# Biblbrox/ViT-Spectre-Experiments

Hardware: AMD Instinct MI355X
Metric: images/sec training, Spectre-ViT-S CIFAR-100 bs512 (higher is better)
Workload: dtype bf16

## Files before the change

### vit-spectre-experiments_amd/csrc/spv_rowops.hip

```cpp
#define SPV_USES_SEED
#include "spv_common.h"

namespace {

constexpr float LN_EPS = 1e-5f;
constexpr int RT = 256;
constexpr int RW = RT / 64;
constexpr int BWD_MAX_WG = 1024;

enum PoolMode { POOL_IDENT = 0, POOL_EXACT = 1, POOL_TABLE = 2, POOL_REPEAT = 3 };

template <int VEC> __device__ __forceinline__ void ldv(const void* base, size_t off, int bf, float (&v)[VEC]);
template <> __device__ __forceinline__ void ldv<4>(const void* base, size_t off, int bf, float (&v)[4]) {
    if (bf) io<bf16_t>::ld4(static_cast<const bf16_t*>(base) + off, v);
    else io<float>::ld4(static_cast<const float*>(base) + off, v);
}
template <> __device__ __forceinline__ void ldv<1>(const void* base, size_t off, int bf, float (&v)[1]) {
    v[0] = bf ? bf2f(static_cast<const bf16_t*>(base)[off]) : static_cast<const float*>(base)[off];
}
template <int VEC> __device__ __forceinline__ void stv(void* base, size_t off, int bf, const float (&v)[VEC]);
template <> __device__ __forceinline__ void stv<4>(void* base, size_t off, int bf, const float (&v)[4]) {
    if (bf) io<bf16_t>::st4(static_cast<bf16_t*>(base) + off, v);
    else io<float>::st4(static_cast<float*>(base) + off, v);
}
// ... 680 lines not shown
#pragma unroll
        for (int j = 0; j < KD; ++j) {
            const unsigned w[4] = {raw[j].x, raw[j].y, raw[j].z, raw[j].w};
            const float d0[4] = {__uint_as_float(da[j].x << 16), __uint_as_float(da[j].x & 0xffff0000u), __uint_as_float(da[j].y << 16),
                                 __uint_as_float(da[j].y & 0xffff0000u)};
            const float d1[4] = {__uint_as_float(dd[j].x << 16), __uint_as_float(dd[j].x & 0xffff0000u), __uint_as_float(dd[j].y << 16),
                                 __uint_as_float(dd[j].y & 0xffff0000u)};
#pragma unroll
            for (int u = 0; u < 4; ++u) {
                const float x0 = __uint_as_float(w[u] << 16), x1 = __uint_as_float(w[u] & 0xffff0000u);
                const float a = bf2f(f2bf((x0 + x1) * r)), d = bf2f(f2bf((x0 - x1) * r));
                xh0[j][u] = (a - mu) * rs;
                xh1[j][u] = (d - mu) * rs;
                acc[0][j][u] += d0[u] * xh0[j][u];
                acc[1][j][u] += d0[u];
                acc[0][KD + j][u] += d1[u] * xh1[j][u];
                acc[1][KD + j][u] += d1[u];
                t0[j][u] = d0[u] * g0[j][u];
                t1[j][u] = d1[u] * g1[j][u];
                s1 += t0[j][u] + t1[j][u];
                s2 += t0[j][u] * xh0[j][u] + t1[j][u] * xh1[j][u];
            }
        }
        const float m1 = wave_sum(s1) * (1.0f / (float)D), m2 = wave_sum(s2) * (1.0f / (float)D);
        bf16_t* orow = dx + (size_t)row * D;
#pragma unroll
        for (int j = 0; j < KD; ++j) {
            const int c = 64 * j + lane;
            const unsigned wr[4] = {res[j].x, res[j].y, res[j].z, res[j].w};
            float o[8];
#pragma unroll
            for (int u = 0; u < 4; ++u) {
                const float ga = bf2f(f2bf(rs * (t0[j][u] - m1 - xh0[j][u] * m2)));
                const float gd = bf2f(f2bf(rs * (t1[j][u] - m1 - xh1[j][u] * m2)));
                o[2 * u] = (ga + gd) * r + __uint_as_float(wr[u] << 16);
                o[2 * u + 1] = (ga - gd) * r + __uint_as_float(wr[u] & 0xffff0000u);
            }
            uint4 t;
            t.x = pack_bf16x2(o[0], o[1]); t.y = pack_bf16x2(o[2], o[3]); t.z = pack_bf16x2(o[4], o[5]); t.w = pack_bf16x2(o[6], o[7]);
            *reinterpret_cast<uint4*>(orow + 8 * c) = t;
        }
    }
    write_partials<4, MAXI, 2>(acc, lds, partials + (size_t)blockIdx.x * 2 * D, D, lane, wave);
}

__global__ __launch_bounds__(FOLD_COLS * FOLD_ROWS) void fold_partials_kernel(const float* __restrict__ partials, float* __restrict__ o0,
                                                                             float* __restrict__ o1, float* __restrict__ o2,
                                                                             int parts, int np, int n, float* __restrict__ o3 = nullptr,
                                                                             float* __restrict__ o4 = nullptr) {
    const FoldJob j{partials, {o0, o1, o2, o3, o4}, parts, np, n};
    fold_partials_block(j, blockIdx.x, threadIdx.x);
}

constexpr int lc_ws(int c, int CO, int CI) { return (c * CI) / CO; }
constexpr int lc_we(int c, int CO, int CI) { return ((c + 1) * CI + CO - 1) / CO; }

template <int CNT> __device__ __forceinline__ void ld_span(const void* base, size_t off, int bf, float (&v)[CNT]) {
#pragma unroll
    for (int q = 0; q < CNT / 4; ++q) {
        float t[4];
        ldv<4>(base, off + 4 * q, bf, t);
#pragma unroll
        for (int u = 0; u < 4; ++u) v[4 * q + u] = t[u];
    }
}
template <int CNT> __device__ __forceinline__ void st_span(void* base, size_t off, int bf, const float (&v)[CNT]) {
#pragma unroll
    for (int q = 0; q < CNT / 4; ++q) {
        float t[4];
#pragma unroll
        for (int u = 0; u < 4; ++u) t[u] = v[4 * q + u];
        stv<4>(base, off + 4 * q, bf, t);
    }
}

template <int CNT, int BF> struct RawSpan;
template <int CNT> struct RawSpan<CNT, 1> { unsigned w[CNT / 2]; };
template <int CNT> struct RawSpan<CNT, 0> { float w[CNT]; };
template <int CNT, int BF> __device__ __forceinline__ void ld_raw(const void* base, size_t off, RawSpan<CNT, BF>& r) {
    if constexpr (BF) {
        const unsigned* p = reinterpret_cast<const unsigned*>(static_cast<const bf16_t*>(base) + off);
#pragma unroll
        for (int i = 0; i < CNT / 2; ++i) r.w[i] = p[i];
    } else {
        const float* p = static_cast<const float*>(base) + off;
#pragma unroll
        for (int i = 0; i < CNT; ++i) r.w[i] = p[i];
    }
}
template <int CNT, int BF> __device__ __forceinline__ void unpack(const RawSpan<CNT, BF>& r, float (&v)[CNT]) {
    if constexpr (BF) {
#pragma unroll
        for (int i = 0; i < CNT / 2; ++i) {
            v[2 * i] = __uint_as_float(r.w[i] << 16);
            v[2 * i + 1] = __uint_as_float(r.w[i] & 0xffff0000u);
        }
    } else {
#pragma unroll
        for (int i = 0; i < CNT; ++i) v[i] = r.w[i];
    }
}

struct TailLn2 {
    const void* res;
    const float* gamma2;
    const float* beta2;
    void* out2;
    float* mean2;
    float* rstd2;
    const void* dout2;
    const void* f3;
    void* ds;
};
__device__ __forceinline__ float round_store(float v, int bf) { return bf ? bf2f(f2bf(v)) : v; }

template <int CO, int CI, bool FASTG, bool LN2>
__global__ __launch_bounds__(RT, 4) void tail_fwd_lc_kernel(const void* __restrict__ h, const void* __restrict__ x,
                                                             const float* __restrict__ gamma, const float* __restrict__ beta,
                                                             void* __restrict__ out, float* __restrict__ mean_o,
                                                             float* __restrict__ rstd_o, int rows, int bf_rt, int out_bf_rt, float p_drop,
                                                             uint64_t seed, TailLn2 ln) {
    constexpr int bf = FASTG ? 1 : 0, out_bf = bf;
    (void)bf_rt; (void)out_bf_rt;
    constexpr int n = 64 * CO, k_in = 64 * CI;
    constexpr float inv_n = 1.0f / (float)n;
    const int lane = threadIdx.x & 63;
    const int wave_g = blockIdx.x * RW + (threadIdx.x >> 6);
    const int nwaves = gridDim.x * RW;
    const float inv_keep = p_drop > 0.0f ? 1.0f / (1.0f - p_drop) : 1.0f;
    const uint64_t seed_l = live_seed(seed);
    float g[CO], b[CO];
    ld_span<CO>(gamma, (size_t)lane * CO, 0, g);
    ld_span<CO>(beta, (size_t)lane * CO, 0, b);
    for (int row = wave_g; row < rows; row += nwaves) {
        RawSpan<CO, bf> r_h, r_res;
        RawSpan<CI, bf> r_x;
        ld_raw<CO, bf>(h, (size_t)row * n + lane * CO, r_h);
        ld_raw<CI, bf>(x, (size_t)row * k_in + lane * CI, r_x);
        if (LN2) ld_raw<CO, bf>(ln.res, (size_t)row * n + lane * CO, r_res);
        float hv[CO], xin[CI];
        unpack<CO, bf>(r_h, hv);
        unpack<CI, bf>(r_x, xin);
        float s = 0.0f;
#pragma unroll
        for (int c = 0; c < CO; ++c) s += hv[c];
        const float mean = wave_sum(s) * inv_n;
        float q = 0.0f;
#pragma unroll
        for (int c = 0; c < CO; ++c) { const float d = hv[c] - mean; q += d * d; }
        const float rstd = rsqrtf(wave_sum(q) * inv_n + LN_EPS);
        const unsigned rkey = p_drop > 0.0f ? dropout_row_key(seed_l, (uint64_t)row) : 0u;
        const unsigned lane_gold = (unsigned)(lane * (CO / 2)) * 0x9e3779b1u;
        float o[CO];
#pragma unroll
        for (int c = 0; c < CO; c += 2) {
            float pv[2];
#pragma unroll
            for (int u = 0; u < 2; ++u) {
                float acc = 0.0f;
#pragma unroll
                for (int j = 0; j < CI; ++j)
                    if (j >= lc_ws(c + u, CO, CI) && j < lc_we(c + u, CO, CI)) acc += xin[j];
                pv[u] = acc * (1.0f / (float)(lc_we(c + u, CO, CI) - lc_ws(c + u, CO, CI)));
            }
            const f32x2 hv2 = {hv[c], hv[c + 1]}, g2 = {g[c], g[c + 1]}, b2 = {b[c], b[c + 1]};
            const f32x2 ln = (hv2 - mean) * (g2 * rstd) + b2;
            f32x2 act, unused;
            if (FASTG) gelu_fast2(ln, act, unused);
            else act = f32x2{gelu_erf(ln.x), gelu_erf(ln.y)};
            o[c] = act.x + pv[0];
            o[c + 1] = act.y + pv[1];
            if (p_drop > 0.0f) {
                o[c] *= dropout_scale_at(rkey + lane_gold, c, p_drop, inv_keep);
                o[c + 1] *= dropout_scale_at(rkey + lane_gold, c + 1, p_drop, inv_keep);
            }
        }
        st_span<CO>(out, (size_t)row * n + lane * CO, out_bf, o);
        if (lane == 0) { mean_o[row] = mean; rstd_o[row] = rstd; }
        if (LN2) {
            float rv[CO], g2[CO], b2[CO];
            unpack<CO, bf>(r_res, rv);
            float sm = 0.0f;
#pragma unroll
            for (int c = 0; c < CO; ++c) { rv[c] += round_store(o[c], out_bf); sm += rv[c]; }
            const float mean2 = wave_sum(sm) * inv_n;
            float q2 = 0.0f;
#pragma unroll
            for (int c = 0; c < CO; ++c) { const float d = rv[c] - mean2; q2 += d * d; }
            const float rstd2 = rsqrtf(wave_sum(q2) * inv_n + LN_EPS);
            ld_span<CO>(ln.gamma2, (size_t)lane * CO, 0, g2);
            ld_span<CO>(ln.beta2, (size_t)lane * CO, 0, b2);
#pragma unroll
            for (int c = 0; c < CO; ++c) rv[c] = (rv[c] - mean2) * rstd2 * g2[c] + b2[c];
            st_span<CO>(ln.out2, (size_t)row * n + lane * CO, bf, rv);
            if (lane == 0) { ln.mean2[row] = mean2; ln.rstd2[row] = rstd2; }
        }
    }
}

struct TailUp {
    const void* src;
    float p_drop;
    uint64_t seed;
};

template <int CO, int CI, bool FASTG, bool LN2>
__global__ __launch_bounds__(RT, 4) void tail_bwd_lc_kernel(const void* __restrict__ dout, const void* __restrict__ h,
                                                             const float* __restrict__ mean_i, const float* __restrict__ rstd_i,
                                                             const float* __restrict__ gamma, const float* __restrict__ beta,
                                                             void* __restrict__ dh, void* __restrict__ dxp, float* __restrict__ partials,
                                                             int rows, int bf_rt, int dout_bf_rt, float p_drop, uint64_t seed,
                                                             const void* __restrict__ dx_add, TailLn2 ln, TailUp up) {
    extern __shared__ __attribute__((aligned(16))) float lds[];
    constexpr int bf = FASTG ? 1 : 0;
    (void)bf_rt; (void)dout_bf_rt;
    constexpr int n = 64 * CO, k_in = 64 * CI, Q = CO / 4;
    constexpr float inv_n = 1.0f / (float)n;
    constexpr int NP = LN2 ? 5 : 3;
    static_assert(CO % 4 == 0, "lane span must be whole float4s");
    const int lane = threadIdx.x & 63, wave = threadIdx.x >> 6;
    const int wave_g = blockIdx.x * RW + wave;
    const int nwaves = gridDim.x * RW;
    const float inv_keep = p_drop > 0.0f ? 1.0f / (1.0f - p_drop) : 1.0f;
    float4* accw = reinterpret_cast<float4*>(lds) + (size_t)wave * NP * Q * 64 + lane;
#pragma unroll
    for (int i = 0; i < NP * Q; ++i) accw[i * 64] = make_float4(0.0f, 0.0f, 0.0f, 0.0f);
    const uint64_t seed_l = live_seed(seed), up_seed_l = live_seed(up.seed);
    for (int row = wave_g; row < rows; row += nwaves) {
        RawSpan<CO, bf> r_h, r_d, r_s, r_t;
        RawSpan<CI, bf> r_u, r_a;
        ld_raw<CO, bf>(LN2 ? ln.dout2 : dout, (size_t)row * n + lane * CO, r_d);
        ld_raw<CO, bf>(h, (size_t)row * n + lane * CO, r_h);
        if (LN2) {
            ld_raw<CO, bf>(ln.f3, (size_t)row * n + lane * CO, r_s);
            ld_raw<CO, bf>(ln.res, (size_t)row * n + lane * CO, r_t);
        }
        constexpr bool WIDE_IN = CI > 16;
        if constexpr (!WIDE_IN) {
            if (!LN2 && up.src != nullptr) ld_raw<CI, bf>(up.src, (size_t)row * k_in + lane * CI, r_u);
            if (dxp != nullptr && dx_add != nullptr) ld_raw<CI, bf>(dx_add, (size_t)row * k_in + lane * CI, r_a);
        }
        const float mean = mean_i[row], rstd = rstd_i[row];
        const unsigned rkey = p_drop > 0.0f ? dropout_row_key(seed_l, (uint64_t)row) : 0u;
        const unsigned lane_gold = (unsigned)(lane * (CO / 2)) * 0x9e3779b1u;
        float hv[CO], dv[CO], dxh[CO];
        unpack<CO, bf>(r_d, dv);
        if (LN2) {
            float sv[CO], tv[CO];
            unpack<CO, bf>(r_s, sv);
            unpack<CO, bf>(r_t, tv);
            const float mean2 = ln.mean2[row], rstd2 = ln.rstd2[row];
            float t1 = 0.0f, t2 = 0.0f;
#pragma unroll
            for (int q = 0; q < Q; ++q) {
                float g2[4];
                ld_span<4>(ln.gamma2, (size_t)lane * CO + 4 * q, 0, g2);
                float4 v3 = accw[(3 * Q + q) * 64], v4 = accw[(4 * Q + q) * 64];
                float a3[4];
#pragma unroll
                for (int e = 0; e < 4; ++e) {
                    const int c = 4 * q + e;
                    const float xh = (sv[c] + tv[c] - mean2) * rstd2;
                    a3[e] = dv[c] * xh;
                    sv[c] = xh;
                    tv[c] = dv[c] * g2[e];
                    t1 += tv[c];
                    t2 += tv[c] * xh;
                }
                v3.x += a3[0]; v3.y += a3[1]; v3.z += a3[2]; v3.w += a3[3];
                v4.x += dv[4 * q]; v4.y += dv[4 * q + 1]; v4.z += dv[4 * q + 2]; v4.w += dv[4 * q + 3];
                accw[(3 * Q + q) * 64] = v3;
                accw[(4 * Q + q) * 64] = v4;
            }
            const float n1 = wave_sum(t1) * inv_n, n2 = wave_sum(t2) * inv_n;
#pragma unroll
            for (int c = 0; c < CO; ++c) dv[c] = round_store(rstd2 * (tv[c] - n1 - sv[c] * n2), bf);
            st_span<CO>(ln.ds, (size_t)row * n + lane * CO, bf, dv);
        } else {
            if (up.src != nullptr) {
                float u[CI];
                unpack<CI, bf>(r_u, u);
                if (up.p_drop > 0.0f) {
                    const unsigned ukey = dropout_row_key(up_seed_l, (uint64_t)row);
                    const float uinv = 1.0f / (1.0f - up.p_drop);
#pragma unroll
                    for (int c = 0; c < CI; ++c) u[c] *= dropout_scale_at(ukey + (unsigned)(lane * (CI / 2)) * 0x9e3779b1u, c, up.p_drop, uinv);
                }
#pragma unroll
                for (int j = 0; j < CO; ++j) {
                    float a = 0.0f;
#pragma unroll
                    for (int c = 0; c < CI; ++c)
                        if (j >= lc_ws(c, CI, CO) && j < lc_we(c, CI, CO)) a += u[c] * (1.0f / (float)(lc_we(c, CI, CO) - lc_ws(c, CI, CO)));
                    dv[j] += a;
                }
            }
        }
        unpack<CO, bf>(r_h, hv);
        f32x2 s1v = {0.0f, 0.0f}, s2v = {0.0f, 0.0f};
#pragma unroll
        for (int q = 0; q < Q; ++q) {
            float g[4], b[4], a0[4], a1[4];
            ld_span<4>(gamma, (size_t)lane * CO + 4 * q, 0, g);
            ld_span<4>(beta, (size_t)lane * CO + 4 * q, 0, b);
#pragma unroll
            for (int e = 0; e < 4; e += 2) {
                const int c = 4 * q + e;
                if (p_drop > 0.0f) {
                    dv[c] *= dropout_scale_at(rkey + lane_gold, c, p_drop, inv_keep);
                    dv[c + 1] *= dropout_scale_at(rkey + lane_gold, c + 1, p_drop, inv_keep);
                }
                const f32x2 hv2 = {hv[c], hv[c + 1]}, g2 = {g[e], g[e + 1]}, b2 = {b[e], b[e + 1]}, dv2 = {dv[c], dv[c + 1]};
                const f32x2 xhat = (hv2 - mean) * rstd;
                f32x2 dgel, unused;
                if (FASTG) gelu_fast2(xhat * g2 + b2, unused, dgel);
                else {
                    const f32x2 pre = xhat * g2 + b2;
                    dgel = f32x2{gelu_erf_grad(pre.x), gelu_erf_grad(pre.y)};
                }
                const f32x2 dln = dv2 * dgel;
                const f32x2 ax = dln * xhat;
                const f32x2 t = dln * g2;
                s1v += t;
                s2v += t * xhat;
                a0[e] = ax.x; a0[e + 1] = ax.y;
                a1[e] = dln.x; a1[e + 1] = dln.y;
                dxh[c] = t.x; dxh[c + 1] = t.y;
            }
            float4 v0 = accw[(0 * Q + q) * 64], v1 = accw[(1 * Q + q) * 64];
            v0.x += a0[0]; v0.y += a0[1]; v0.z += a0[2]; v0.w += a0[3];
            v1.x += a1[0]; v1.y += a1[1]; v1.z += a1[2]; v1.w += a1[3];
            accw[(0 * Q + q) * 64] = v0;
            accw[(1 * Q + q) * 64] = v1;
            __builtin_amdgcn_sched_barrier(0);
        }
        const float m1 = wave_sum(s1v.x + s1v.y) * inv_n, m2 = wave_sum(s2v.x + s2v.y) * inv_n;
        float o[CO];
#pragma unroll
        for (int q = 0; q < Q; ++q) {
            float4 v2 = accw[(2 * Q + q) * 64];
#pragma unroll
            for (int e = 0; e < 4; e += 2) {
                const int c = 4 * q + e;
                const f32x2 hv2 = {hv[c], hv[c + 1]}, t2 = {dxh[c], dxh[c + 1]};
                const f32x2 o2 = (t2 - m1 - (hv2 - mean) * (rstd * m2)) * rstd;
                o[c] = o2.x;
                o[c + 1] = o2.y;
            }
            v2.x += o[4 * q]; v2.y += o[4 * q + 1]; v2.z += o[4 * q + 2]; v2.w += o[4 * q + 3];
            accw[(2 * Q + q) * 64] = v2;
        }
        st_span<CO>(dh, (size_t)row * n + lane * CO, bf, o);
        if (dxp == nullptr) continue;
        if constexpr (WIDE_IN) {
#pragma unroll
            for (int j0 = 0; j0 < CI; j0 += 8) {
                float dxc[8];
#pragma unroll
                for (int jj = 0; jj < 8; ++jj) {
                    const int j = j0 + jj;
                    float a = 0.0f;
#pragma unroll
                    for (int c = 0; c < CO; ++c)
                        if (j >= lc_ws(c, CO, CI) && j < lc_we(c, CO, CI)) a += dv[c] * (1.0f / (float)(lc_we(c, CO, CI) - lc_ws(c, CO, CI)));
                    dxc[jj] = a;
                }
                if (dx_add != nullptr) {
                    RawSpan<8, bf> ra;
                    ld_raw<8, bf>(dx_add, (size_t)row * k_in + lane * CI + j0, ra);
                    float ad[8];
                    unpack<8, bf>(ra, ad);
#pragma unroll
                    for (int jj = 0; jj < 8; ++jj) dxc[jj] += ad[jj];
                }
                st_span<8>(dxp, (size_t)row * k_in + lane * CI + j0, bf, dxc);
            }
            continue;
        }
        float dx[CI];
#pragma unroll
        for (int j = 0; j < CI; ++j) {
            float a = 0.0f;
#pragma unroll
            for (int c = 0; c < CO; ++c)
                if (j >= lc_ws(c, CO, CI) && j < lc_we(c, CO, CI)) a += dv[c] * (1.0f / (float)(lc_we(c, CO, CI) - lc_ws(c, CO, CI)));
            dx[j] = a;
        }
        if (dx_add != nullptr) {
            float ad[CI];
            unpack<CI, bf>(r_a, ad);
#pragma unroll
            for (int j = 0; j < CI; ++j) dx[j] += ad[j];
        }
        st_span<CI>(dxp, (size_t)row * k_in + lane * CI, bf, dx);
    }
    __syncthreads();
    float* slab = partials + (size_t)blockIdx.x * NP * n;
    for (int i = threadIdx.x; i < NP * n; i += blockDim.x) {
        const int p = i / n, col = i - p * n;
        const int l = col / CO, r = col - l * CO;
        const int off = (((p * Q + (r >> 2)) * 64 + l) << 2) + (r & 3);
        float v = lds[off];
#pragma unroll
        for (int w = 1; w < RW; ++w) v += lds[w * NP * n + off];
        slab[i] = v;
    }
}

constexpr int WCO = 12, WR = 4, WCI = WCO / WR;
template <int BF, bool FASTG>
__global__ __launch_bounds__(RT) void tail_wide_fwd_kernel(const void* __restrict__ h, const void* __restrict__ x, const float* __restrict__ gamma,
                                                           const float* __restrict__ beta, void* __restrict__ out, float* __restrict__ mean_o,
                                                           float* __restrict__ rstd_o, int rows, float p_drop, uint64_t seed) {
    constexpr int n = RW * 64 * WCO, k_in = n / WR;
    constexpr float inv_n = 1.0f / (float)n;
    __shared__ float red[2][2][RW];
    const int lane = threadIdx.x & 63, wave = threadIdx.x >> 6;
    const int col0 = (wave * 64 + lane) * WCO, in0 = (wave * 64 + lane) * WCI;
    const float inv_keep = p_drop > 0.0f ? 1.0f / (1.0f - p_drop) : 1.0f;
    const uint64_t seed_l = live_seed(seed);
    float g[WCO], b[WCO];
    ld_span<WCO>(gamma, col0, 0, g);
    ld_span<WCO>(beta, col0, 0, b);
    int par = 0;
    for (int row = blockIdx.x; row < rows; row += gridDim.x, par ^= 1) {
        RawSpan<WCO, BF> r_h;
        ld_raw<WCO, BF>(h, (size_t)row * n + col0, r_h);
        float xv[WCI];
#pragma unroll
        for (int j = 0; j < WCI; ++j) xv[j] = BF ? bf2f(static_cast<const bf16_t*>(x)[(size_t)row * k_in + in0 + j]) : static_cast<const float*>(x)[(size_t)row * k_in + in0 + j];
        float hv[WCO];
        unpack<WCO, BF>(r_h, hv);
        float sm = 0.0f;
#pragma unroll
        for (int c = 0; c < WCO; ++c) sm += hv[c];
        sm = wave_sum(sm);
        if (lane == 0) red[par][0][wave] = sm;
        __syncthreads();
        float tot = 0.0f;
#pragma unroll
        for (int w = 0; w < RW; ++w) tot += red[par][0][w];
        const float mean = tot * inv_n;
        float q = 0.0f;
#pragma unroll
        for (int c = 0; c < WCO; ++c) { const float d = hv[c] - mean; q += d * d; }
        q = wave_sum(q);
        if (lane == 0) red[par][1][wave] = q;
// ... 120 lines not shown
            else if (cfg.vec == 4 && cfg.maxi == 3) hipLaunchKernelGGL((KERNEL<4, 3, false>), grid, dim3(RT), lds_bytes, st, __VA_ARGS__);   \
            else if (cfg.vec == 4 && cfg.maxi == 4) hipLaunchKernelGGL((KERNEL<4, 4, false>), grid, dim3(RT), lds_bytes, st, __VA_ARGS__);   \
            else if (cfg.vec == 4 && cfg.maxi == 12) hipLaunchKernelGGL((KERNEL<4, 12, false>), grid, dim3(RT), lds_bytes, st, __VA_ARGS__); \
            else if (cfg.vec == 4 && cfg.maxi == 16) hipLaunchKernelGGL((KERNEL<4, 16, false>), grid, dim3(RT), lds_bytes, st, __VA_ARGS__); \
            else hipLaunchKernelGGL((KERNEL<1, 16, false>), grid, dim3(RT), lds_bytes, st, __VA_ARGS__);        \
        }                                                                                                      \
    } while (0)

struct RowCfg { int vec, maxi; };
inline bool pick_cfg(int n, RowCfg& c) {
    if (n % 4 == 0) {
        const int ni = cdiv(n, 256);
        c.vec = 4;
        if (ni <= 2) c.maxi = 2; else if (ni <= 3) c.maxi = 3; else if (ni <= 4) c.maxi = 4;
        else if (ni <= 12) c.maxi = 12; else if (ni <= 16) c.maxi = 16; else return false;
        return true;
    }
    if (n <= 1024) { c.vec = 1; c.maxi = 16; return true; }
    return false;
}

#define ROW_DISPATCH(cfg, KERNEL, grid, lds_bytes, st, ...)                                                    \
    do {                                                                                                       \
        if (cfg.vec == 4 && cfg.maxi == 2) hipLaunchKernelGGL((KERNEL<4, 2>), grid, dim3(RT), lds_bytes, st, __VA_ARGS__);        \
        else if (cfg.vec == 4 && cfg.maxi == 3) hipLaunchKernelGGL((KERNEL<4, 3>), grid, dim3(RT), lds_bytes, st, __VA_ARGS__);   \
        else if (cfg.vec == 4 && cfg.maxi == 4) hipLaunchKernelGGL((KERNEL<4, 4>), grid, dim3(RT), lds_bytes, st, __VA_ARGS__);   \
        else if (cfg.vec == 4 && cfg.maxi == 12) hipLaunchKernelGGL((KERNEL<4, 12>), grid, dim3(RT), lds_bytes, st, __VA_ARGS__); \
        else if (cfg.vec == 4 && cfg.maxi == 16) hipLaunchKernelGGL((KERNEL<4, 16>), grid, dim3(RT), lds_bytes, st, __VA_ARGS__); \
        else hipLaunchKernelGGL((KERNEL<1, 16>), grid, dim3(RT), lds_bytes, st, __VA_ARGS__);                  \
    } while (0)

inline int check_dtype(int d) { return d == SPV_F32 || d == SPV_BF16; }
inline int pool_mode_of(int n, int k_in) {
    return k_in == n ? POOL_IDENT : (k_in % n == 0 ? POOL_EXACT : (n % k_in == 0 ? POOL_REPEAT : POOL_TABLE));
}

}

extern "C" int64_t spv_rowop_partial_floats(int n) { return (int64_t)BWD_MAX_WG * 3 * n; }
extern "C" int spv_tail_bwd_parts(int rows) { return std::min(cdiv(rows, RW), BWD_MAX_WG); }

extern "C" int spv_spectre_tail_fwd(const void* h, const void* x, const float* gamma, const float* beta, void* out,
                                    float* mean, float* rstd, int rows, int n, int k_in, int dtype, int out_dtype,
                                    float p_drop, uint64_t seed, void* stream) {
    SPV_CHECK(rows > 0 && n > 0 && k_in > 0, "spv_spectre_tail_fwd: empty");
    SPV_CHECK(check_dtype(dtype) && check_dtype(out_dtype), "spv_spectre_tail_fwd: bad dtype");
    SPV_CHECK(p_drop >= 0.0f && p_drop < 1.0f, "spv_spectre_tail_fwd: p_drop=%f", p_drop);
    RowCfg cfg;
    SPV_CHECK(pick_cfg(n, cfg), "spv_spectre_tail_fwd: unsupported row length %d", n);
    hipStream_t st = static_cast<hipStream_t>(stream);
    SPV_CHECK((int64_t)n * k_in < (1ll << 31), "spv_spectre_tail_fwd: n*k_in too large");
    {
        const int fast = dtype == SPV_BF16, bfl = dtype == SPV_BF16, obf = out_dtype == SPV_BF16;
        constexpr int fwd_wgs = 2048;
        dim3 lgrid(std::min(cdiv(rows, RW), fwd_wgs));
#define LC_FWD(CO, CI)                                                                                                        \
        if (n == 64 * CO && k_in == 64 * CI && obf == bfl) {                                                                  \
            SPV_COUNT_PATH(SPV_PATH_TAIL_LC); \
            if (fast) hipLaunchKernelGGL((tail_fwd_lc_kernel<CO, CI, true, false>), lgrid, dim3(RT), 0, static_cast<hipStream_t>(stream), h, x, gamma, beta, out, mean, rstd, rows, bfl, obf, p_drop, seed, TailLn2{}); \
            else hipLaunchKernelGGL((tail_fwd_lc_kernel<CO, CI, false, false>), lgrid, dim3(RT), 0, static_cast<hipStream_t>(stream), h, x, gamma, beta, out, mean, rstd, rows, bfl, obf, p_drop, seed, TailLn2{});    \
            SPV_LAUNCH_CHECK("spv_spectre_tail_fwd(lc)");                                                                     \
            return 0;                                                                                                         \
        }
        LC_FWD(12, 8)
        LC_FWD(8, 12)
        LC_FWD(8, 8)
        LC_FWD(12, 48)
#undef LC_FWD
    }
    if (n == RW * 64 * WCO && k_in * WR == n && (out_dtype == SPV_BF16) == (dtype == SPV_BF16) &&
        (((uintptr_t)h | (uintptr_t)out | (uintptr_t)gamma | (uintptr_t)beta) & 15) == 0) {
        const dim3 wgrid(std::min(rows, 2048));
        if (dtype == SPV_BF16) hipLaunchKernelGGL((tail_wide_fwd_kernel<1, true>), wgrid, dim3(RT), 0, st, h, x, gamma, beta, out, mean, rstd, rows, p_drop, seed);
        else hipLaunchKernelGGL((tail_wide_fwd_kernel<0, false>), wgrid, dim3(RT), 0, st, h, x, gamma, beta, out, mean, rstd, rows, p_drop, seed);
        SPV_LAUNCH_CHECK("spv_spectre_tail_fwd(wide)");
        return 0;
    }
    const int pm = pool_mode_of(n, k_in);
    dim3 grid(std::min(cdiv(rows, RW), 2048));
    const size_t lds_f = pm == POOL_TABLE ? ((size_t)2 * n + (size_t)RW * k_in) * sizeof(float)
                         : (pm == POOL_EXACT && (k_in / n) % 4 == 0 ? (size_t)RW * (k_in / 4) * sizeof(float) : 0);
    SPV_CHECK(lds_f <= 64 * 1024, "spv_spectre_tail_fwd: n=%d k_in=%d needs %zu bytes of LDS", n, k_in, lds_f);
    TAIL_DISPATCH(cfg, dtype == SPV_BF16, tail_fwd_kernel, grid, lds_f, st, h, x, gamma, beta, out, mean,
                 rstd, rows, n, k_in, dtype == SPV_BF16, out_dtype == SPV_BF16, p_drop, seed, pm);
    SPV_LAUNCH_CHECK("spv_spectre_tail_fwd");
    return 0;
}

static int tail_bwd_impl(const void* dout, const void* h, const float* mean, const float* rstd, const float* gamma, const float* beta,
                         void* dh, void* dx_pool, float* dgamma, float* dbeta, float* dbias, float* partials, int rows, int n,
                         int k_in, int dtype, int dout_dtype, float p_drop, uint64_t seed, const void* dx_add, void* stream, TailUp up) {
    SPV_CHECK(rows > 0 && n > 0 && k_in > 0, "spv_spectre_tail_bwd: empty");
    SPV_CHECK(up.src == nullptr || (n == 768 && k_in == 512), "spv_spectre_tail_bwd_up: only the 512 -> 768 layer takes the skip gradient of the layer above");
    SPV_CHECK(check_dtype(dtype) && check_dtype(dout_dtype), "spv_spectre_tail_bwd: bad dtype");
    RowCfg cfg;
    SPV_CHECK(pick_cfg(n, cfg), "spv_spectre_tail_bwd: unsupported row length %d", n);
    hipStream_t st = static_cast<hipStream_t>(stream);
    SPV_CHECK((int64_t)n * k_in < (1ll << 31), "spv_spectre_tail_bwd: n*k_in too large");
    {
        const int fast = dtype == SPV_BF16, bfl = dtype == SPV_BF16, dbf = dout_dtype == SPV_BF16;
        const int lwgs = std::min(cdiv(rows, RW), BWD_MAX_WG);
        const int k_lc = (dx_pool == nullptr && up.src == nullptr) ? n : k_in;
#define LC_BWD(CO, CI)                                                                                                        \
        if (n == 64 * CO && k_lc == 64 * CI && (dbf == bfl || up.src != nullptr)) {                                          \
            SPV_CHECK(dbf == bfl, "spv_spectre_tail_bwd_up: dout must have the tensors' dtype");                              \
            hipStream_t lst = static_cast<hipStream_t>(stream);                                                               \
            SPV_COUNT_PATH(up.src ? SPV_PATH_TAIL_UP : SPV_PATH_TAIL_LC); \
            if (fast) hipLaunchKernelGGL((tail_bwd_lc_kernel<CO, CI, true, false>), dim3(lwgs), dim3(RT), (size_t)RW * 3 * n * sizeof(float), lst, dout, h, mean, rstd, gamma, beta, dh, dx_pool, partials, rows, bfl, dbf, p_drop, seed, dx_add, TailLn2{}, up); \
// ... 19 lines not shown
        SPV_LAUNCH_CHECK("spv_spectre_tail_bwd(wide)");
        if (dgamma != nullptr) hipLaunchKernelGGL(fold_partials_kernel, dim3(cdiv(3 * n, FOLD_COLS)), dim3(FOLD_COLS * FOLD_ROWS), 0, st, partials, dgamma, dbeta, dbias, wwgs, 3, n);
        SPV_LAUNCH_CHECK("spv_spectre_tail_bwd(wide fold)");
        return 0;
    }
    const int pm = pool_mode_of(n, k_in);
    const int wgs = std::min(cdiv(rows, RW), BWD_MAX_WG);
    const size_t lds = (size_t)3 * n * sizeof(float) + (pm == POOL_TABLE ? (size_t)(2 * k_in + n + RW * n) * sizeof(int) : 0);
    SPV_CHECK(lds <= 64 * 1024, "spv_spectre_tail_bwd: n=%d k_in=%d needs %zu bytes of LDS", n, k_in, lds);
    TAIL_DISPATCH(cfg, dtype == SPV_BF16, tail_bwd_kernel, dim3(wgs), lds, st, dout, h, mean, rstd, gamma, beta, dh,
                 dx_pool, partials, rows, n, k_in, dtype == SPV_BF16, dout_dtype == SPV_BF16, p_drop, seed, pm, dx_add);
    SPV_LAUNCH_CHECK("spv_spectre_tail_bwd");
    if (dgamma != nullptr) hipLaunchKernelGGL(fold_partials_kernel, dim3(cdiv(3 * n, FOLD_COLS)), dim3(FOLD_COLS * FOLD_ROWS), 0, st, partials, dgamma, dbeta, dbias, wgs, 3, n);
    SPV_LAUNCH_CHECK("spv_spectre_tail_bwd(fold)");
    return 0;
}

extern "C" int spv_spectre_tail_bwd(const void* dout, const void* h, const float* mean, const float* rstd,
                                    const float* gamma, const float* beta, void* dh, void* dx_pool, float* dgamma,
                                    float* dbeta, float* dbias, float* partials, int rows, int n, int k_in, int dtype,
                                    int dout_dtype, float p_drop, uint64_t seed, const void* dx_add, void* stream) {
    return tail_bwd_impl(dout, h, mean, rstd, gamma, beta, dh, dx_pool, dgamma, dbeta, dbias, partials, rows, n, k_in, dtype, dout_dtype,
                         p_drop, seed, dx_add, stream, TailUp{nullptr, 0.0f, 0});
}

extern "C" int spv_tail_up_supported(int n, int k_in, int dtype) {
    return (n == 768 && k_in == 512 && check_dtype(dtype)) ? 1 : 0;
}

extern "C" int spv_spectre_tail_bwd_up(const void* dout, const void* h, const float* mean, const float* rstd, const float* gamma,
                                       const float* beta, void* dh, void* dx_pool, float* dgamma, float* dbeta, float* dbias,
                                       float* partials, int rows, int n, int k_in, int dtype, int dout_dtype, float p_drop,
                                       uint64_t seed, const void* dx_add, const void* up_src, float up_p_drop, uint64_t up_seed,
                                       void* stream) {
    SPV_CHECK(up_src != nullptr && spv_tail_up_supported(n, k_in, dtype), "spv_spectre_tail_bwd_up: unsupported shape %d -> %d", k_in, n);
    SPV_CHECK(up_p_drop >= 0.0f && up_p_drop < 1.0f, "spv_spectre_tail_bwd_up: up_p_drop=%f", up_p_drop);
    return tail_bwd_impl(dout, h, mean, rstd, gamma, beta, dh, dx_pool, dgamma, dbeta, dbias, partials, rows, n, k_in, dtype, dout_dtype,
                         p_drop, seed, dx_add, stream, TailUp{up_src, up_p_drop, up_seed});
}

extern "C" int spv_tail_ln_supported(int n, int k_in, int dtype) {
    return (n == 512 && k_in == 768 && check_dtype(dtype)) ? 1 : 0;
}
extern "C" int64_t spv_tail_ln_partial_floats(int n) { return (int64_t)BWD_MAX_WG * 5 * n; }

extern "C" int spv_spectre_tail_ln_fwd(const void* h, const void* x, const float* gamma, const float* beta, void* out, float* mean,
                                       float* rstd, const void* res, const float* gamma2, const float* beta2, void* out2, float* mean2,
                                       float* rstd2, int rows, int n, int k_in, int dtype, float p_drop, uint64_t seed, void* stream) {
    SPV_CHECK(rows > 0 && spv_tail_ln_supported(n, k_in, dtype), "spv_spectre_tail_ln_fwd: unsupported shape %d -> %d / dtype %d", k_in, n, dtype);
    SPV_CHECK(p_drop >= 0.0f && p_drop < 1.0f, "spv_spectre_tail_ln_fwd: p_drop=%f", p_drop);
    SPV_CHECK(h && x && gamma && beta && out && mean && rstd && res && gamma2 && beta2 && out2 && mean2 && rstd2, "spv_spectre_tail_ln_fwd: null pointer");
    const int bfl = dtype == SPV_BF16;
    TailLn2 ln{res, gamma2, beta2, out2, mean2, rstd2, nullptr, nullptr, nullptr};
    dim3 lgrid(std::min(cdiv(rows, RW), 2048));
    hipStream_t st = static_cast<hipStream_t>(stream);
    SPV_COUNT_PATH(SPV_PATH_TAIL_LN);
    if (bfl) hipLaunchKernelGGL((tail_fwd_lc_kernel<8, 12, true, true>), lgrid, dim3(RT), 0, st, h, x, gamma, beta, out, mean, rstd, rows, bfl, bfl, p_drop, seed, ln);
    else hipLaunchKernelGGL((tail_fwd_lc_kernel<8, 12, false, true>), lgrid, dim3(RT), 0, st, h, x, gamma, beta, out, mean, rstd, rows, bfl, bfl, p_drop, seed, ln);
    SPV_LAUNCH_CHECK("spv_spectre_tail_ln_fwd");
    return 0;
}

extern "C" int spv_spectre_tail_ln_bwd(const void* dout2, const void* f3, const void* res, const float* mean2, const float* rstd2,
                                       const float* gamma2, void* ds, float* dgamma2, float* dbeta2, const void* h, const float* mean,
                                       const float* rstd, const float* gamma, const float* beta, void* dh, void* dx_pool, float* dgamma,
                                       float* dbeta, float* dbias, float* partials, int rows, int n, int k_in, int dtype, float p_drop,
                                       uint64_t seed, void* stream) {
    SPV_CHECK(rows > 0 && spv_tail_ln_supported(n, k_in, dtype), "spv_spectre_tail_ln_bwd: unsupported shape %d -> %d / dtype %d", k_in, n, dtype);
    SPV_CHECK(dout2 && f3 && res && mean2 && rstd2 && gamma2 && ds && h && mean && rstd && gamma && beta && dh && partials,
              "spv_spectre_tail_ln_bwd: null pointer");
    SPV_CHECK((dgamma && dbeta && dbias && dgamma2 && dbeta2) || (!dgamma && !dbeta && !dbias && !dgamma2 && !dbeta2),
              "spv_spectre_tail_ln_bwd: the five parameter gradients are given together, or all NULL (the caller folds the partials)");
    const int bfl = dtype == SPV_BF16;
    TailLn2 ln{res, gamma2, nullptr, nullptr, const_cast<float*>(mean2), const_cast<float*>(rstd2), dout2, f3, ds};
    const int lwgs = std::min(cdiv(rows, RW), BWD_MAX_WG);
    const size_t lds = (size_t)RW * 5 * n * sizeof(float);
    hipStream_t st = static_cast<hipStream_t>(stream);
    SPV_COUNT_PATH(SPV_PATH_TAIL_LN);
    if (bfl) hipLaunchKernelGGL((tail_bwd_lc_kernel<8, 12, true, true>), dim3(lwgs), dim3(RT), lds, st, nullptr, h, mean, rstd, gamma, beta, dh, dx_pool, partials, rows, bfl, bfl, p_drop, seed, nullptr, ln, TailUp{nullptr, 0.0f, 0});
    else hipLaunchKernelGGL((tail_bwd_lc_kernel<8, 12, false, true>), dim3(lwgs), dim3(RT), lds, st, nullptr, h, mean, rstd, gamma, beta, dh, dx_pool, partials, rows, bfl, bfl, p_drop, seed, nullptr, ln, TailUp{nullptr, 0.0f, 0});
    SPV_LAUNCH_CHECK("spv_spectre_tail_ln_bwd");
    if (dgamma != nullptr) hipLaunchKernelGGL(fold_partials_kernel, dim3(cdiv(5 * n, FOLD_COLS)), dim3(FOLD_COLS * FOLD_ROWS), 0, st, partials, dgamma, dbeta, dbias, lwgs, 5, n, dgamma2, dbeta2);
    SPV_LAUNCH_CHECK("spv_spectre_tail_ln_bwd(fold)");
    return 0;
}

extern "C" int spv_haar_ln_supported(int dim, int dtype) {
    return (dtype == SPV_BF16 && (dim == 512 || dim == 1024)) ? 1 : 0;
}

extern "C" int spv_haar_ln_fwd(const void* x, const float* gamma, const float* beta, void* out, float* mean, float* rstd, int rows, int dim,
                               int dtype, void* stream) {
    SPV_CHECK(rows > 0 && spv_haar_ln_supported(dim, dtype), "spv_haar_ln_fwd: unsupported dim %d / dtype %d", dim, dtype);
    SPV_CHECK(x && gamma && beta && out && mean && rstd, "spv_haar_ln_fwd: null pointer");
    SPV_CHECK((((uintptr_t)x | (uintptr_t)out | (uintptr_t)gamma | (uintptr_t)beta) & 15) == 0, "spv_haar_ln_fwd: pointers must be 16-byte aligned");
    hipStream_t st = static_cast<hipStream_t>(stream);
    const dim3 grid(std::min(cdiv(rows, RW), 2048));
    if (dim == 512) hipLaunchKernelGGL((haar_ln_fwd_kernel<1>), grid, dim3(RT), 0, st, (const bf16_t*)x, gamma, beta, (bf16_t*)out, mean, rstd, rows);
    else hipLaunchKernelGGL((haar_ln_fwd_kernel<2>), grid, dim3(RT), 0, st, (const bf16_t*)x, gamma, beta, (bf16_t*)out, mean, rstd, rows);
    SPV_LAUNCH_CHECK("spv_haar_ln_fwd");
    return 0;
}

extern "C" int spv_haar_ln_bwd(const void* dout, const void* x, const float* mean, const float* rstd, const float* gamma, void* dx,
                               float* dgamma, float* dbeta, float* partials, int rows, int dim, int dtype, void* stream) {
    SPV_CHECK(rows > 0 && spv_haar_ln_supported(dim, dtype), "spv_haar_ln_bwd: unsupported dim %d / dtype %d", dim, dtype);
    SPV_CHECK(dout && x && mean && rstd && gamma && dx && partials && ((dgamma != nullptr) == (dbeta != nullptr)), "spv_haar_ln_bwd: null pointer");
// ... 63 lines not shown
```

Baseline: 322,900.

## Software-pipeline row loads in Spectre tail LC fwd/bwd kernels with uniform row pointers

Restructures the tail forward and backward LC kernels to double-buffer row inputs, issuing the next row's global loads before computing the current row so memory latency overlaps with LayerNorm/GELU/pooling math. Row base pointers are made wave-uniform via readfirstlane so addressing can use scalar registers. The forward kernel stages gamma/beta (and the second LN's parameters) in LDS instead of holding them in registers. The forward grid cap drops from 2048 to 1280 workgroups. The cost is higher register pressure from two live row buffers, which may lower occupancy, plus a clamped redundant load on the final iteration.

After: 317,200. 0.983x the previous value.

```diff
diff --git a/vit-spectre-experiments_amd/csrc/spv_rowops.hip b/vit-spectre-experiments_amd/csrc/spv_rowops.hip
--- a/vit-spectre-experiments_amd/csrc/spv_rowops.hip
+++ b/vit-spectre-experiments_amd/csrc/spv_rowops.hip
@@ -756,6 +756,10 @@
     fold_partials_block(j, blockIdx.x, threadIdx.x);
 }
 
+template <bool FASTG> constexpr bool LC_PIPE = FASTG;
+constexpr int LC_BWD_PF = 0;
+constexpr int LC_FWD_OCC = 4;
+constexpr int LC_FWD_WGS = 1280;
 constexpr int lc_ws(int c, int CO, int CI) { return (c * CI) / CO; }
 constexpr int lc_we(int c, int CO, int CI) { return ((c + 1) * CI + CO - 1) / CO; }
 
@@ -791,6 +795,35 @@
 #pragma unroll
         for (int i = 0; i < CNT; ++i) r.w[i] = p[i];
     }
+}
+__device__ __forceinline__ const char* uniform_ptr(const char* p) {
+    const uint64_t v = reinterpret_cast<uint64_t>(p);
+    const uint32_t lo = __builtin_amdgcn_readfirstlane(static_cast<uint32_t>(v));
+    const uint32_t hi = __builtin_amdgcn_readfirstlane(static_cast<uint32_t>(v >> 32));
+    typedef const __attribute__((address_space(1))) char* global_cptr;
+    return (const char*)(global_cptr)((static_cast<uint64_t>(hi) << 32) | lo);
+}
+template <int CNT, int BF> __device__ __forceinline__ void ld_raw_row(const void* base, size_t row_off, unsigned lane_off, RawSpan<CNT, BF>& r) {
+    constexpr unsigned ES = BF ? 2 : 4;
+    const char* rp = uniform_ptr(static_cast<const char*>(base) + row_off * ES);
+    if constexpr (BF) {
+        const unsigned* p = reinterpret_cast<const unsigned*>(rp + lane_off * ES);
+#pragma unroll
+        for (int i = 0; i < CNT / 2; ++i) r.w[i] = p[i];
+    } else {
+        const float* p = reinterpret_cast<const float*>(rp + lane_off * ES);
+#pragma unroll
+        for (int i = 0; i < CNT; ++i) r.w[i] = p[i];
+    }
+}
+template <int CNT> __device__ __forceinline__ void st_span_row(void* base, size_t row_off, unsigned lane_off, int bf, const float (&v)[CNT]) {
+    const unsigned es = bf ? 2 : 4;
+    char* rp = const_cast<char*>(uniform_ptr(static_cast<char*>(base) + row_off * es));
+    st_span<CNT>(rp + lane_off * es, 0, bf, v);
+}
+__device__ __forceinline__ void ld_f4_lane(const float* base, unsigned elem_off, float (&v)[4]) {
+    const float4 t = *reinterpret_cast<const float4*>(uniform_ptr(reinterpret_cast<const char*>(base)) + elem_off * 4u);
+    v[0] = t.x; v[1] = t.y; v[2] = t.z; v[3] = t.w;
 }
 template <int CNT, int BF> __device__ __forceinline__ void unpack(const RawSpan<CNT, BF>& r, float (&v)[CNT]) {
     if constexpr (BF) {
@@ -819,7 +852,7 @@
 __device__ __forceinline__ float round_store(float v, int bf) { return bf ? bf2f(f2bf(v)) : v; }
 
 template <int CO, int CI, bool FASTG, bool LN2>
-__global__ __launch_bounds__(RT, 4) void tail_fwd_lc_kernel(const void* __restrict__ h, const void* __restrict__ x,
+__global__ __launch_bounds__(RT, LC_FWD_OCC) void tail_fwd_lc_kernel(const void* __restrict__ h, const void* __restrict__ x,
                                                              const float* __restrict__ gamma, const float* __restrict__ beta,
                                                              void* __restrict__ out, float* __restrict__ mean_o,
                                                              float* __restrict__ rstd_o, int rows, int bf_rt, int out_bf_rt, float p_drop,
@@ -829,19 +862,28 @@
     constexpr int n = 64 * CO, k_in = 64 * CI;
     constexpr float inv_n = 1.0f / (float)n;
     const int lane = threadIdx.x & 63;
-    const int wave_g = blockIdx.x * RW + (threadIdx.x >> 6);
+    const int wave_g = blockIdx.x * RW + __builtin_amdgcn_readfirstlane(threadIdx.x >> 6);
     const int nwaves = gridDim.x * RW;
     const float inv_keep = p_drop > 0.0f ? 1.0f / (1.0f - p_drop) : 1.0f;
     const uint64_t seed_l = live_seed(seed);
-    float g[CO], b[CO];
-    ld_span<CO>(gamma, (size_t)lane * CO, 0, g);
-    ld_span<CO>(beta, (size_t)lane * CO, 0, b);
-    for (int row = wave_g; row < rows; row += nwaves) {
-        RawSpan<CO, bf> r_h, r_res;
-        RawSpan<CI, bf> r_x;
-        ld_raw<CO, bf>(h, (size_t)row * n + lane * CO, r_h);
-        ld_raw<CI, bf>(x, (size_t)row * k_in + lane * CI, r_x);
-        if (LN2) ld_raw<CO, bf>(ln.res, (size_t)row * n + lane * CO, r_res);
+    __shared__ __attribute__((aligned(16))) float gb[(LN2 ? 4 : 2) * n];
+    for (int i = threadIdx.x; i < n; i += RT) {
+        gb[i] = gamma[i]; gb[n + i] = beta[i];
+        if constexpr (LN2) { gb[2 * n + i] = ln.gamma2[i]; gb[3 * n + i] = ln.beta2[i]; }
+    }
+    __syncthreads();
+    auto lds4 = [&](int arr, int c, float (&v)[4]) __attribute__((always_inline)) {
+        const float4 t = *reinterpret_cast<const float4*>(&gb[arr * n + lane * CO + c]);
+        v[0] = t.x; v[1] = t.y; v[2] = t.z; v[3] = t.w;
+    };
+    if (wave_g >= rows) return;
+    auto load_row = [&](int r, RawSpan<CO, bf>& r_h, RawSpan<CI, bf>& r_x, RawSpan<CO, bf>& r_res) __attribute__((always_inline)) {
+        r = __builtin_amdgcn_readfirstlane(r < rows ? r : rows - 1);
+        ld_raw_row<CO, bf>(h, (size_t)r * n, (unsigned)lane * CO, r_h);
+        ld_raw_row<CI, bf>(x, (size_t)r * k_in, (unsigned)lane * CI, r_x);
+        if (LN2) ld_raw_row<CO, bf>(ln.res, (size_t)r * n, (unsigned)lane * CO, r_res);
+    };
+    auto do_row = [&](const int row, const RawSpan<CO, bf>& r_h, const RawSpan<CI, bf>& r_x, const RawSpan<CO, bf>& r_res) __attribute__((always_inline)) {
         float hv[CO], xin[CI];
         unpack<CO, bf>(r_h, hv);
         unpack<CI, bf>(r_x, xin);
@@ -856,8 +898,10 @@
         const unsigned rkey = p_drop > 0.0f ? dropout_row_key(seed_l, (uint64_t)row) : 0u;
         const unsigned lane_gold = (unsigned)(lane * (CO / 2)) * 0x9e3779b1u;
         float o[CO];
+        float g[4], b[4];
 #pragma unroll
         for (int c = 0; c < CO; c += 2) {
+            if (c % 4 == 0) { lds4(0, c, g); lds4(1, c, b); }
             float pv[2];
 #pragma unroll
             for (int u = 0; u < 2; ++u) {
@@ -867,7 +911,7 @@
                     if (j >= lc_ws(c + u, CO, CI) && j < lc_we(c + u, CO, CI)) acc += xin[j];
                 pv[u] = acc * (1.0f / (float)(lc_we(c + u, CO, CI) - lc_ws(c + u, CO, CI)));
             }
-            const f32x2 hv2 = {hv[c], hv[c + 1]}, g2 = {g[c], g[c + 1]}, b2 = {b[c], b[c + 1]};
+            const f32x2 hv2 = {hv[c], hv[c + 1]}, g2 = {g[c % 4], g[c % 4 + 1]}, b2 = {b[c % 4], b[c % 4 + 1]};
             const f32x2 ln = (hv2 - mean) * (g2 * rstd) + b2;
             f32x2 act, unused;
             if (FASTG) gelu_fast2(ln, act, unused);
@@ -879,10 +923,10 @@
                 o[c + 1] *= dropout_scale_at(rkey + lane_gold, c + 1, p_drop, inv_keep);
             }
         }
-        st_span<CO>(out, (size_t)row * n + lane * CO, out_bf, o);
+        st_span_row<CO>(out, (size_t)row * n, (unsigned)lane * CO, out_bf, o);
         if (lane == 0) { mean_o[row] = mean; rstd_o[row] = rstd; }
         if (LN2) {
-            float rv[CO], g2[CO], b2[CO];
+            float rv[CO];
             unpack<CO, bf>(r_res, rv);
             float sm = 0.0f;
 #pragma unroll
@@ -892,13 +936,38 @@
 #pragma unroll
             for (int c = 0; c < CO; ++c) { const float d = rv[c] - mean2; q2 += d * d; }
             const float rstd2 = rsqrtf(wave_sum(q2) * inv_n + LN_EPS);
-            ld_span<CO>(ln.gamma2, (size_t)lane * CO, 0, g2);
-            ld_span<CO>(ln.beta2, (size_t)lane * CO, 0, b2);
-#pragma unroll
-            for (int c = 0; c < CO; ++c) rv[c] = (rv[c] - mean2) * rstd2 * g2[c] + b2[c];
-            st_span<CO>(ln.out2, (size_t)row * n + lane * CO, bf, rv);
+#pragma unroll
+            for (int q = 0; q < CO / 4; ++q) {
+                float g2[4], b2[4];
+                lds4(2, 4 * q, g2);
+                lds4(3, 4 * q, b2);
+#pragma unroll
+                for (int e = 0; e < 4; ++e) rv[4 * q + e] = (rv[4 * q + e] - mean2) * rstd2 * g2[e] + b2[e];
+            }
+            st_span_row<CO>(ln.out2, (size_t)row * n, (unsigned)lane * CO, bf, rv);
             if (lane == 0) { ln.mean2[row] = mean2; ln.rstd2[row] = rstd2; }
         }
+    };
+    RawSpan<CO, bf> a_h, a_res, b_h, b_res;
+    RawSpan<CI, bf> a_x, b_x;
+    int row = wave_g;
+    if constexpr (!LC_PIPE<FASTG>) {
+        for (; row < rows; row += nwaves) {
+            load_row(row, a_h, a_x, a_res);
+            do_row(row, a_h, a_x, a_res);
+        }
+        return;
+    }
+    load_row(row, a_h, a_x, a_res);
+    for (;;) {
+        load_row(row + nwaves, b_h, b_x, b_res);
+        do_row(row, a_h, a_x, a_res);
+        row += nwaves;
+        if (row >= rows) break;
+        load_row(row + nwaves, a_h, a_x, a_res);
+        do_row(row, b_h, b_x, b_res);
+        row += nwaves;
+        if (row >= rows) break;
     }
 }
 
@@ -922,7 +991,7 @@
     constexpr float inv_n = 1.0f / (float)n;
     constexpr int NP = LN2 ? 5 : 3;
     static_assert(CO % 4 == 0, "lane span must be whole float4s");
-    const int lane = threadIdx.x & 63, wave = threadIdx.x >> 6;
+    const int lane = threadIdx.x & 63, wave = __builtin_amdgcn_readfirstlane(threadIdx.x >> 6);
     const int wave_g = blockIdx.x * RW + wave;
     const int nwaves = gridDim.x * RW;
     const float inv_keep = p_drop > 0.0f ? 1.0f / (1.0f - p_drop) : 1.0f;
@@ -930,21 +999,31 @@
 #pragma unroll
     for (int i = 0; i < NP * Q; ++i) accw[i * 64] = make_float4(0.0f, 0.0f, 0.0f, 0.0f);
     const uint64_t seed_l = live_seed(seed), up_seed_l = live_seed(up.seed);
-    for (int row = wave_g; row < rows; row += nwaves) {
-        RawSpan<CO, bf> r_h, r_d, r_s, r_t;
-        RawSpan<CI, bf> r_u, r_a;
-        ld_raw<CO, bf>(LN2 ? ln.dout2 : dout, (size_t)row * n + lane * CO, r_d);
-        ld_raw<CO, bf>(h, (size_t)row * n + lane * CO, r_h);
+    constexpr bool WIDE_IN = CI > 16;
+    struct RowIn {
+        RawSpan<CO, bf> h, d, s, t;
+        RawSpan<CI, bf> u, a;
+        float mean, rstd, mean2, rstd2;
+    };
+    auto load_row = [&](int r, RowIn& in) __attribute__((always_inline)) {
+        r = __builtin_amdgcn_readfirstlane(r < rows ? r : rows - 1);
+        ld_raw_row<CO, bf>(LN2 ? ln.dout2 : dout, (size_t)r * n, (unsigned)lane * CO, in.d);
+        ld_raw_row<CO, bf>(h, (size_t)r * n, (unsigned)lane * CO, in.h);
         if (LN2) {
-            ld_raw<CO, bf>(ln.f3, (size_t)row * n + lane * CO, r_s);
-            ld_raw<CO, bf>(ln.res, (size_t)row * n + lane * CO, r_t);
-        }
-        constexpr bool WIDE_IN = CI > 16;
+            ld_raw_row<CO, bf>(ln.f3, (size_t)r * n, (unsigned)lane * CO, in.s);
+            ld_raw_row<CO, bf>(ln.res, (size_t)r * n, (unsigned)lane * CO, in.t);
+        }
         if constexpr (!WIDE_IN) {
-            if (!LN2 && up.src != nullptr) ld_raw<CI, bf>(up.src, (size_t)row * k_in + lane * CI, r_u);
-            if (dxp != nullptr && dx_add != nullptr) ld_raw<CI, bf>(dx_add, (size_t)row * k_in + lane * CI, r_a);
-        }
-        const float mean = mean_i[row], rstd = rstd_i[row];
+            if (!LN2 && up.src != nullptr) ld_raw_row<CI, bf>(up.src, (size_t)r * k_in, (unsigned)lane * CI, in.u);
+            if (dxp != nullptr && dx_add != nullptr) ld_raw_row<CI, bf>(dx_add, (size_t)r * k_in, (unsigned)lane * CI, in.a);
+        }
+        in.mean = mean_i[r]; in.rstd = rstd_i[r];
+        if (LN2) { in.mean2 = ln.mean2[r]; in.rstd2 = ln.rstd2[r]; }
+    };
+    auto do_row = [&](const int row, const RowIn& in, RowIn& nxt) __attribute__((always_inline)) {
+        const RawSpan<CO, bf>&r_h = in.h, &r_d = in.d, &r_s = in.s, &r_t = in.t;
+        const RawSpan<CI, bf>&r_u = in.u, &r_a = in.a;
+        const float mean = in.mean, rstd = in.rstd;
         const unsigned rkey = p_drop > 0.0f ? dropout_row_key(seed_l, (uint64_t)row) : 0u;
         const unsigned lane_gold = (unsigned)(lane * (CO / 2)) * 0x9e3779b1u;
         float hv[CO], dv[CO], dxh[CO];
@@ -953,12 +1032,12 @@
             float sv[CO], tv[CO];
             unpack<CO, bf>(r_s, sv);
             unpack<CO, bf>(r_t, tv);
-            const float mean2 = ln.mean2[row], rstd2 = ln.rstd2[row];
+            const float mean2 = in.mean2, rstd2 = in.rstd2;
             float t1 = 0.0f, t2 = 0.0f;
 #pragma unroll
             for (int q = 0; q < Q; ++q) {
                 float g2[4];
-                ld_span<4>(ln.gamma2, (size_t)lane * CO + 4 * q, 0, g2);
+                ld_f4_lane(ln.gamma2, (unsigned)(lane * CO + 4 * q), g2);
                 float4 v3 = accw[(3 * Q + q) * 64], v4 = accw[(4 * Q + q) * 64];
                 float a3[4];
 #pragma unroll
@@ -979,7 +1058,7 @@
             const float n1 = wave_sum(t1) * inv_n, n2 = wave_sum(t2) * inv_n;
 #pragma unroll
             for (int c = 0; c < CO; ++c) dv[c] = round_store(rstd2 * (tv[c] - n1 - sv[c] * n2), bf);
-            st_span<CO>(ln.ds, (size_t)row * n + lane * CO, bf, dv);
+            st_span_row<CO>(ln.ds, (size_t)row * n, (unsigned)lane * CO, bf, dv);
         } else {
             if (up.src != nullptr) {
                 float u[CI];
@@ -1005,8 +1084,9 @@
 #pragma unroll
         for (int q = 0; q < Q; ++q) {
             float g[4], b[4], a0[4], a1[4];
-            ld_span<4>(gamma, (size_t)lane * CO + 4 * q, 0, g);
-            ld_span<4>(beta, (size_t)lane * CO + 4 * q, 0, b);
+            ld_f4_lane(gamma, (unsigned)(lane * CO + 4 * q), g);
+            ld_f4_lane(beta, (unsigned)(lane * CO + 4 * q), b);
+            if (LC_PIPE<FASTG> && LC_BWD_PF == 0 && q == Q - 1) load_row(row + nwaves, nxt);
 #pragma unroll
             for (int e = 0; e < 4; e += 2) {
                 const int c = 4 * q + e;
@@ -1038,6 +1118,7 @@
             accw[(1 * Q + q) * 64] = v1;
             __builtin_amdgcn_sched_barrier(0);
         }
+        if (LC_PIPE<FASTG> && LC_BWD_PF == 1) load_row(row + nwaves, nxt);
         const float m1 = wave_sum(s1v.x + s1v.y) * inv_n, m2 = wave_sum(s2v.x + s2v.y) * inv_n;
         float o[CO];
 #pragma unroll
@@ -1054,8 +1135,8 @@
             v2.x += o[4 * q]; v2.y += o[4 * q + 1]; v2.z += o[4 * q + 2]; v2.w += o[4 * q + 3];
             accw[(2 * Q + q) * 64] = v2;
         }
-        st_span<CO>(dh, (size_t)row * n + lane * CO, bf, o);
-        if (dxp == nullptr) continue;
+        st_span_row<CO>(dh, (size_t)row * n, (unsigned)lane * CO, bf, o);
+        if (dxp == nullptr) return;
         if constexpr (WIDE_IN) {
 #pragma unroll
             for (int j0 = 0; j0 < CI; j0 += 8) {
@@ -1079,7 +1160,7 @@
                 }
                 st_span<8>(dxp, (size_t)row * k_in + lane * CI + j0, bf, dxc);
             }
-            continue;
+            return;
         }
         float dx[CI];
 #pragma unroll
@@ -1096,7 +1177,21 @@
 #pragma unroll
             for (int j = 0; j < CI; ++j) dx[j] += ad[j];
         }
-        st_span<CI>(dxp, (size_t)row * k_in + lane * CI, bf, dx);
+        st_span_row<CI>(dxp, (size_t)row * k_in, (unsigned)lane * CI, bf, dx);
+    };
+    if (wave_g < rows) {
+        RowIn ra, rb;
+        int row = wave_g;
+        load_row(row, ra);
+        for (;;) {
+            do_row(row, ra, rb);
+            row += nwaves;
+            if (row >= rows) break;
+            if constexpr (!LC_PIPE<FASTG>) { load_row(row, ra); continue; }
+            do_row(row, rb, ra);
+            row += nwaves;
+            if (row >= rows) break;
+        }
     }
     __syncthreads();
     float* slab = partials + (size_t)blockIdx.x * NP * n;
@@ -1323,8 +1418,7 @@
     SPV_CHECK((int64_t)n * k_in < (1ll << 31), "spv_spectre_tail_fwd: n*k_in too large");
     {
         const int fast = dtype == SPV_BF16, bfl = dtype == SPV_BF16, obf = out_dtype == SPV_BF16;
-        constexpr int fwd_wgs = 2048;
-        dim3 lgrid(std::min(cdiv(rows, RW), fwd_wgs));
+        dim3 lgrid(std::min(cdiv(rows, RW), LC_FWD_WGS));
 #define LC_FWD(CO, CI)                                                                                                        \
         if (n == 64 * CO && k_in == 64 * CI && obf == bfl) {                                                                  \
             SPV_COUNT_PATH(SPV_PATH_TAIL_LC); \
@@ -1450,7 +1544,7 @@
     SPV_CHECK(h && x && gamma && beta && out && mean && rstd && res && gamma2 && beta2 && out2 && mean2 && rstd2, "spv_spectre_tail_ln_fwd: null pointer");
     const int bfl = dtype == SPV_BF16;
     TailLn2 ln{res, gamma2, beta2, out2, mean2, rstd2, nullptr, nullptr, nullptr};
-    dim3 lgrid(std::min(cdiv(rows, RW), 2048));
+    dim3 lgrid(std::min(cdiv(rows, RW), LC_FWD_WGS));
     hipStream_t st = static_cast<hipStream_t>(stream);
     SPV_COUNT_PATH(SPV_PATH_TAIL_LN);
     if (bfl) hipLaunchKernelGGL((tail_fwd_lc_kernel<8, 12, true, true>), lgrid, dim3(RT), 0, st, h, x, gamma, beta, out, mean, rstd, rows, bfl, bfl, p_drop, seed, ln);
```
